# zju3dv/pats

Hardware: AMD Instinct MI355X
Metric: image-pairs/sec (coarse+fine OT) on 640x480 MegaDepth; OT iters/sec per pair (higher is better)
Workload: dtype f32 (contractions: fp32 operands split into fp16 hi + lo, three exact-product MFMA passes, fp32 accumulate)

## Files before the change

include/pats_amd.h:

```cpp
#ifndef PATS_AMD_H
#define PATS_AMD_H

#include <stddef.h>
#include <stdint.h>

#ifdef __cplusplus
extern "C" {
#endif

typedef void* pats_stream_t;

enum {
    PATS_OK = 0,
    PATS_ERR_INVALID = 1,
    PATS_ERR_UNSUPPORTED = 2,
    PATS_ERR_LAUNCH = 3,
    PATS_ERR_NO_DEVICE = 4
};

enum { PATS_SINKHORN_AUTO = 0, PATS_SINKHORN_LOG = 1, PATS_SINKHORN_KERNEL = 2 };

const char* pats_version(void);
#define PATS_ABI_VERSION 8
int pats_abi_version(void);
const char* pats_last_error(void);
int pats_device_count(void);
int pats_set_sinkhorn_mode(int mode);
int pats_set_fine_fused(int on);

int pats_set_third_gather(int mode);

int pats_sinkhorn_fallbacks(int64_t* count, int reset);

int pats_cost_f32(const float* d0, const float* d1, int64_t batch, int D, int n, int m, float* out,
                  pats_stream_t stream);

size_t pats_sinkhorn_workspace_bytes(int64_t batch, int M, int N);
int pats_sinkhorn_f32(const float* Z, int64_t batch, int M, int N, const float* log_mu,
                      const float* log_nu, int iters, float* out, void* workspace,
                      size_t workspace_bytes, pats_stream_t stream);

size_t pats_ot_workspace_bytes(int64_t batch, int M, int N);
int pats_log_optimal_transport_f32(const float* scores, int64_t batch, int m, int n,
                                   const float* alpha, const float* ns, int iters, float* Z,
                                   void* workspace, size_t workspace_bytes, pats_stream_t stream);

size_t pats_ot2_workspace_bytes(int64_t batch, int m, int n);
int pats_log_optimal_transport2_flags_f32(const float* scores, int64_t batch, int m, int n,
                                          const float* one, const float* ns, int iters, float bias_k,
                                          float* Z, uint8_t* col_nomatch, void* workspace,
                                          size_t workspace_bytes, pats_stream_t stream);
int pats_log_optimal_transport2_f32(const float* scores, int64_t batch, int m, int n,
                                    const float* one, const float* ns, int iters, float bias_k,
                                    float* Z, void* workspace, size_t workspace_bytes,
                                    pats_stream_t stream);

int pats_cost_ot_f32(const float* d0, const float* d1, int64_t batch, int D, int n, int m,
                     int variant, const float* scalar, const float* ns, int iters, float bias_k,
                     float* Z, void* workspace, size_t workspace_bytes, pats_stream_t stream);
size_t pats_cost_ot_workspace_bytes(int64_t batch, int D, int n, int m, int variant);
int pats_cost_ot_flags_f32(const float* d0, const float* d1, int64_t batch, int D, int n, int m,
                           int variant, const float* scalar, const float* ns, int iters, float bias_k,
                           float* Z, uint8_t* col_nomatch, void* workspace, size_t workspace_bytes,
                           pats_stream_t stream);

int pats_set_cost_ot_mid_event(void* event);

int pats_cost_ot_flags_counted_f32(const float* d0, const float* d1, int64_t batch_cap, const int64_t* batch_dev,
                                   int D, int n, int m, int variant, const float* scalar, const float* ns, int iters,
                                   float bias_k, float* Z, uint8_t* col_nomatch, void* workspace,
                                   size_t workspace_bytes, pats_stream_t stream);

int pats_colmass_sqrt_f32(const float* Z, int64_t batch, int M, int N, float* out,
                          pats_stream_t stream);
int pats_colmass_flags_f32(const float* Z, int64_t batch, int M, int N, float* out, uint8_t* col_nomatch,
                           pats_stream_t stream);
int pats_dustbin_bias_inplace_f32(float* Z, int64_t batch, int M, int N, float k,
                                  pats_stream_t stream);
int pats_exp_f32(const float* Z, int64_t count, float* out, pats_stream_t stream);

int pats_argmax_f32(const float* Z, int64_t batch, int M, int N, int64_t* row_arg,
                    int64_t* col_arg, pats_stream_t stream);

int pats_iterative_expand_f32(const float* P, int input_is_log, int64_t batch, int M, int N,
                              const float* scalex, const float* scaley, int lim3, int h, int w,
                              float lower_bound, int iter_num, float* whole_cost, float* core_cost,
                              float* average_point, float* x_scale, float* y_scale, int64_t* bound,
                              uint8_t* row_nomatch, pats_stream_t stream);

int pats_iterative_expand_counted_f32(const float* P, int input_is_log, int64_t batch_cap, const int64_t* batch_dev,
                                      int M, int N, const float* scalex, const float* scaley, int lim3, int h, int w,
                                      float lower_bound, int iter_num, float* whole_cost, float* core_cost,
                                      float* average_point, float* x_scale, float* y_scale, int64_t* bound,
                                      uint8_t* row_nomatch, pats_stream_t stream);

int pats_split_patches(const int32_t* sum_cycle_host, int height, int width, int max_once_used,
                       int64_t* second_layer_set, int64_t* third_layer_set);
int pats_split_patches_device(const int32_t* sum_cycle, int64_t pairs, int height, int width,
                              int max_once_used, int64_t* second_layer_set, int64_t* third_layer_set,
                              int32_t* cycle_num, pats_stream_t stream);

int pats_compute_imgs_bounds_f32(const float* x_scale, const float* y_scale,
                                 const float* average_point, const uint8_t* if_nomatching, int Np,
                                 int height, int width, int img, int64_t* bound5, int64_t* K_out,
                                 float* x_scale_new, float* y_scale_new, float* average_new,
                                 pats_stream_t stream);

int pats_left_crops_f32(const float* left, int n_img, int H, int W, const int64_t* bound5, int64_t K,
                        int height, int width, float* out, pats_stream_t stream);

int pats_compute_imgs_bounds_batch_f32(const float* x_scale, const float* y_scale, const float* average_point,
                                       const uint8_t* if_nomatching, int n_img, int Np, int height, int width,
                                       int64_t* bound5, int64_t* K_img, int64_t* K_total, float* x_scale_new,
                                       float* y_scale_new, float* average_new, pats_stream_t stream);
int pats_left_crops_counted_f32(const float* left, int n_img, int H, int W, const int64_t* bound5,
                                int64_t K_cap, const int64_t* K_dev, int height, int width, float* out,
                                pats_stream_t stream);

int pats_tensor_resize_f32(const float* input, int n_img, int C, int Hp, int Wp,
                           const int64_t* bound, int64_t K, float* out, int32_t* status,
                           pats_stream_t stream);
int pats_tensor_resize_hwc_f32(const float* right, int n_img, int H, int W, int margin,
                               const int64_t* bound, int64_t K, float* out, int32_t* status,
                               pats_stream_t stream);
int pats_tensor_resize_hwc_counted_f32(const float* right, int n_img, int H, int W, int margin,
                                       const int64_t* bound, int64_t K_cap, const int64_t* K_dev, float* out,
                                       int32_t* status, pats_stream_t stream);

int pats_compute_result_f32(const float* scores, int input_is_log, int64_t P, const float* scale_x,
                            const float* scale_y, const int64_t* p_s, const int64_t* p_t,
                            int outdoor, float* mkpts0_f, float* mkpts1_f, float* whole_loss,
                            float* label, uint8_t* if_matching1, pats_stream_t stream);
int pats_compute_result_ws_f32(const float* scores, int input_is_log, int64_t P, const float* scale_x,
                               const float* scale_y, const int64_t* p_s, const int64_t* p_t,
                               int outdoor, float* mkpts0_f, float* mkpts1_f, float* whole_loss,
                               float* label, uint8_t* if_matching1, void* workspace, size_t workspace_bytes,
                               pats_stream_t stream);

int pats_fine_descriptors_f32(const float* feat0, const float* feat1, const float* feat2,
                              const float* title, const float* rubbish, int64_t B, float* desc,
                              pats_stream_t stream);

int pats_fine_descriptors_counted_f32(const float* feat0, const float* feat1, const float* feat2,
                                      const float* title, const float* rubbish, int64_t B_cap,
                                      const int64_t* B_dev, int channels_last, float* desc, pats_stream_t stream);

int pats_third_descriptors_f32(const float* feat_f0, const float* feat_f1, const float* mkpts0_c,
                               const float* mkpts1_c, const int64_t* b_ids, const float* kenc,
                               const float* rubbish, int64_t P, int64_t B, float* out0, float* out1,
                               int64_t* p_s_out, int64_t* p_t_out, pats_stream_t stream);

int pats_third_level_f32(const float* feat0, const float* feat1, int64_t P, int D, const float* scale,
                         const float* scale_x, const float* scale_y, const int64_t* p_s,
                         const int64_t* p_t, int iters, int outdoor, float* mkpts0_f, float* mkpts1_f,
                         float* label, uint8_t* if_matching1, float* Z_out, pats_stream_t stream);

int pats_third_descriptors_counted_f32(const float* feat_f0, const float* feat_f1, const float* mkpts0_c,
                                       const float* mkpts1_c, const int64_t* b_ids, const float* kenc,
                                       const float* rubbish, int64_t P_cap, const int64_t* P_dev, int64_t B,
                                       float* out0, float* out1, int64_t* p_s_out, int64_t* p_t_out,
                                       pats_stream_t stream);
int pats_third_level_counted_f32(const float* feat0, const float* feat1, int64_t P_cap, const int64_t* P_dev, int D,
                                 const float* scale, const float* scale_x, const float* scale_y, const int64_t* p_s,
                                 const int64_t* p_t, int iters, int outdoor, float* mkpts0_f, float* mkpts1_f,
                                 float* label, uint8_t* if_matching1, pats_stream_t stream);

int pats_fine_descriptors_nhwc_f32(const float* feat0, const float* feat1, const float* feat2,
                                   const float* title, const float* rubbish, int64_t B, float* desc,
                                   pats_stream_t stream);
int pats_third_descriptors_nhwc_f32(const float* feat_f0, const float* feat_f1, const float* mkpts0_c,
                                    const float* mkpts1_c, const int64_t* b_ids, const float* kenc,
                                    const float* rubbish, int64_t P_cap, const int64_t* P_dev, int64_t B,
                                    float* out0, float* out1, int64_t* p_s_out, int64_t* p_t_out,
                                    pats_stream_t stream);

typedef enum { PATS_MAP_F32 = 0, PATS_MAP_F16 = 1, PATS_MAP_BF16 = 2 } pats_map_dtype_t;
int pats_fine_descriptors_typed(const void* feat0, const void* feat1, const void* feat2, pats_map_dtype_t dtype,
                                int channels_last, const float* title, const float* rubbish, int64_t B_cap,
                                const int64_t* B_dev, float* desc, pats_stream_t stream);
int pats_third_descriptors_typed(const void* feat_f0, const void* feat_f1, pats_map_dtype_t dtype, int channels_last,
                                 const float* mkpts0_c, const float* mkpts1_c, const int64_t* b_ids, const float* kenc,
                                 const float* rubbish, int64_t P_cap, const int64_t* P_dev, int64_t B, float* out0,
                                 float* out1, int64_t* p_s_out, int64_t* p_t_out, pats_stream_t stream);
// ... 206 lines not shown
```

pats_amd/_lib.py:

```python
import ctypes
import os

_HERE = os.path.dirname(os.path.abspath(__file__))
LIB_PATH = os.path.join(_HERE, "libpats_amd.so")
if os.environ.get("PATS_AMD_DIAG_LIB", "") not in ("", "0"):
    _sfx = os.environ["PATS_AMD_DIAG_LIB"]
    LIB_PATH = os.path.join(_HERE, "libpats_amd_diag%s.so" % ("" if _sfx == "1" else _sfx))

c_void_p, c_int, c_i64, c_f, c_size = (ctypes.c_void_p, ctypes.c_int, ctypes.c_int64, ctypes.c_float,
                                       ctypes.c_size_t)

ABI_VERSION = 8



class PairTable(ctypes.Structure):
    _fields_ = [("pairs", ctypes.c_int64), ("shape_host", c_void_p), ("cell_base_host", c_void_p), ("shape", c_void_p),
                ("cell_base", c_void_p), ("img_base", c_void_p)]


_TAB = ctypes.POINTER(PairTable)


class CropFormat(ctypes.Structure):
    _fields_ = [("dtype", ctypes.c_int32), ("layout", ctypes.c_int32), ("normalize", ctypes.c_int32),
                ("mean", ctypes.c_float * 3), ("std", ctypes.c_float * 3)]


_FMT = ctypes.POINTER(CropFormat)

SIGNATURES = {
    "pats_version": (ctypes.c_char_p, []),
    "pats_abi_version": (c_int, []),
    "pats_last_error": (ctypes.c_char_p, []),
    "pats_device_count": (c_int, []),
    "pats_set_sinkhorn_mode": (c_int, [c_int]),
    "pats_set_fine_fused": (c_int, [c_int]),
    "pats_set_third_gather": (c_int, [c_int]),
    "pats_sinkhorn_fallbacks": (c_int, [ctypes.POINTER(ctypes.c_int64), c_int]),
    "pats_set_gnn_redo_mode": (c_int, [c_int]),
    "pats_gnn_overflows": (c_int, [ctypes.POINTER(ctypes.c_int64), c_int]),
    "pats_cost_f32": (c_int, [c_void_p, c_void_p, c_i64, c_int, c_int, c_int, c_void_p, c_void_p]),
    "pats_sinkhorn_workspace_bytes": (c_size, [c_i64, c_int, c_int]),
    "pats_sinkhorn_f32": (c_int, [c_void_p, c_i64, c_int, c_int, c_void_p, c_void_p, c_int, c_void_p,
                                  c_void_p, c_size, c_void_p]),
    "pats_ot_workspace_bytes": (c_size, [c_i64, c_int, c_int]),
    "pats_log_optimal_transport_f32": (c_int, [c_void_p, c_i64, c_int, c_int, c_void_p, c_void_p, c_int,
                                               c_void_p, c_void_p, c_size, c_void_p]),
    "pats_ot2_workspace_bytes": (c_size, [c_i64, c_int, c_int]),
    "pats_log_optimal_transport2_f32": (c_int, [c_void_p, c_i64, c_int, c_int, c_void_p, c_void_p, c_int,
                                                c_f, c_void_p, c_void_p, c_size, c_void_p]),
    "pats_cost_ot_f32": (c_int, [c_void_p, c_void_p, c_i64, c_int, c_int, c_int, c_int, c_void_p,
                                 c_void_p, c_int, c_f, c_void_p, c_void_p, c_size, c_void_p]),
    "pats_cost_ot_flags_f32": (c_int, [c_void_p, c_void_p, c_i64, c_int, c_int, c_int, c_int, c_void_p,
                                       c_void_p, c_int, c_f, c_void_p, c_void_p, c_void_p, c_size, c_void_p]),
    "pats_set_cost_ot_mid_event": (c_int, [c_void_p]),
    "pats_cost_ot_flags_counted_f32": (c_int, [c_void_p, c_void_p, c_i64, c_void_p, c_int, c_int, c_int, c_int, c_void_p,
                                               c_void_p, c_int, c_f, c_void_p, c_void_p, c_void_p, c_size, c_void_p]),
    "pats_iterative_expand_counted_f32": (c_int, [c_void_p, c_int, c_i64, c_void_p, c_int, c_int, c_void_p, c_void_p, c_int,
                                                  c_int, c_int, c_f, c_int, c_void_p, c_void_p, c_void_p,
                                                  c_void_p, c_void_p, c_void_p, c_void_p, c_void_p]),
    "pats_fine_descriptors_counted_f32": (c_int, [c_void_p, c_void_p, c_void_p, c_void_p, c_void_p, c_i64, c_void_p, c_int,
                                                  c_void_p, c_void_p]),
    "pats_log_optimal_transport2_flags_f32": (c_int, [c_void_p, c_i64, c_int, c_int, c_void_p, c_void_p, c_int,
                                                      c_f, c_void_p, c_void_p, c_void_p, c_size, c_void_p]),
    "pats_colmass_flags_f32": (c_int, [c_void_p, c_i64, c_int, c_int, c_void_p, c_void_p, c_void_p]),
    "pats_cost_ot_workspace_bytes": (c_size, [c_i64, c_int, c_int, c_int, c_int]),
    "pats_colmass_sqrt_f32": (c_int, [c_void_p, c_i64, c_int, c_int, c_void_p, c_void_p]),
    "pats_dustbin_bias_inplace_f32": (c_int, [c_void_p, c_i64, c_int, c_int, c_f, c_void_p]),
    "pats_exp_f32": (c_int, [c_void_p, c_i64, c_void_p, c_void_p]),
    "pats_argmax_f32": (c_int, [c_void_p, c_i64, c_int, c_int, c_void_p, c_void_p, c_void_p]),
    "pats_iterative_expand_f32": (c_int, [c_void_p, c_int, c_i64, c_int, c_int, c_void_p, c_void_p, c_int,
                                          c_int, c_int, c_f, c_int, c_void_p, c_void_p, c_void_p,
                                          c_void_p, c_void_p, c_void_p, c_void_p, c_void_p]),
    "pats_split_patches": (c_int, [c_void_p, c_int, c_int, c_int, c_void_p, c_void_p]),
    "pats_split_patches_device": (c_int, [c_void_p, c_i64, c_int, c_int, c_int, c_void_p, c_void_p, c_void_p, c_void_p]),
    "pats_compute_imgs_bounds_batch_f32": (c_int, [c_void_p, c_void_p, c_void_p, c_void_p, c_int, c_int, c_int, c_int,
                                                   c_void_p, c_void_p, c_void_p, c_void_p, c_void_p, c_void_p, c_void_p]),
    "pats_left_crops_counted_f32": (c_int, [c_void_p, c_int, c_int, c_int, c_void_p, c_i64, c_void_p, c_int, c_int,
                                            c_void_p, c_void_p]),
    "pats_tensor_resize_hwc_counted_f32": (c_int, [c_void_p, c_int, c_int, c_int, c_int, c_void_p, c_i64, c_void_p,
                                                   c_void_p, c_void_p, c_void_p]),
    "pats_compute_imgs_bounds_f32": (c_int, [c_void_p, c_void_p, c_void_p, c_void_p, c_int, c_int, c_int,
                                             c_int, c_void_p, c_void_p, c_void_p, c_void_p, c_void_p,
                                             c_void_p]),
    "pats_left_crops_f32": (c_int, [c_void_p, c_int, c_int, c_int, c_void_p, c_i64, c_int, c_int, c_void_p,
                                    c_void_p]),
    "pats_tensor_resize_f32": (c_int, [c_void_p, c_int, c_int, c_int, c_int, c_void_p, c_i64, c_void_p,
                                       c_void_p, c_void_p]),
    "pats_tensor_resize_hwc_f32": (c_int, [c_void_p, c_int, c_int, c_int, c_int, c_void_p, c_i64,
                                           c_void_p, c_void_p, c_void_p]),
    "pats_compute_result_f32": (c_int, [c_void_p, c_int, c_i64, c_void_p, c_void_p, c_void_p, c_void_p,
                                        c_int, c_void_p, c_void_p, c_void_p, c_void_p, c_void_p,
                                        c_void_p]),
    "pats_compute_result_ws_f32": (c_int, [c_void_p, c_int, c_i64, c_void_p, c_void_p, c_void_p, c_void_p,
                                           c_int, c_void_p, c_void_p, c_void_p, c_void_p, c_void_p,
                                           c_void_p, c_size, c_void_p]),
    "pats_fine_descriptors_f32": (c_int, [c_void_p, c_void_p, c_void_p, c_void_p, c_void_p, c_i64, c_void_p, c_void_p]),
    "pats_third_descriptors_f32": (c_int, [c_void_p, c_void_p, c_void_p, c_void_p, c_void_p, c_void_p, c_void_p,
                                           c_i64, c_i64, c_void_p, c_void_p, c_void_p, c_void_p, c_void_p]),
    "pats_third_level_f32": (c_int, [c_void_p, c_void_p, c_i64, c_int, c_void_p, c_void_p, c_void_p, c_void_p,
                                     c_void_p, c_int, c_int, c_void_p, c_void_p, c_void_p, c_void_p, c_void_p,
                                     c_void_p]),
    "pats_third_descriptors_counted_f32": (c_int, [c_void_p, c_void_p, c_void_p, c_void_p, c_void_p, c_void_p, c_void_p,
                                                   c_i64, c_void_p, c_i64, c_void_p, c_void_p, c_void_p, c_void_p, c_void_p]),
    "pats_fine_descriptors_nhwc_f32": (c_int, [c_void_p, c_void_p, c_void_p, c_void_p, c_void_p, c_i64, c_void_p, c_void_p]),
    "pats_third_descriptors_nhwc_f32": (c_int, [c_void_p, c_void_p, c_void_p, c_void_p, c_void_p, c_void_p, c_void_p,
                                                c_i64, c_void_p, c_i64, c_void_p, c_void_p, c_void_p, c_void_p, c_void_p]),
    "pats_fine_descriptors_typed": (c_int, [c_void_p, c_void_p, c_void_p, c_int, c_int, c_void_p, c_void_p, c_i64, c_void_p,
                                            c_void_p, c_void_p]),
    "pats_third_descriptors_typed": (c_int, [c_void_p, c_void_p, c_int, c_int, c_void_p, c_void_p, c_void_p, c_void_p, c_void_p,
                                             c_i64, c_void_p, c_i64, c_void_p, c_void_p, c_void_p, c_void_p, c_void_p]),
    "pats_third_level_counted_f32": (c_int, [c_void_p, c_void_p, c_i64, c_void_p, c_int, c_void_p, c_void_p, c_void_p,
                                             c_void_p, c_void_p, c_int, c_int, c_void_p, c_void_p, c_void_p, c_void_p,
                                             c_void_p]),
    "pats_cost_typed": (c_int, [c_void_p, c_void_p, c_int, c_i64, c_int, c_int, c_int, c_void_p, c_void_p]),
    "pats_cost_ot_typed": (c_int, [c_void_p, c_void_p, c_int, c_i64, c_void_p, c_int, c_int, c_int, c_int, c_void_p, c_void_p,
                                   c_int, c_f, c_void_p, c_void_p, c_void_p, c_size, c_void_p]),
    "pats_third_level_typed": (c_int, [c_void_p, c_void_p, c_int, c_i64, c_void_p, c_int, c_void_p, c_void_p, c_void_p, c_void_p,
                                       c_void_p, c_int, c_int, c_void_p, c_void_p, c_void_p, c_void_p, c_void_p, c_void_p]),
    "pats_chunk_rows_workspace_bytes": (c_size, [c_i64, c_int]),
    "pats_chunk_rows_device": (c_int, [c_void_p, c_i64, c_int, c_int, c_int, c_int, c_i64] + [c_void_p] * 13 +
                               [c_size, c_void_p]),
    "pats_profile_marker": (c_int, [c_int, c_void_p]),
    "pats_stream_create_cu_mask": (c_int, [c_void_p, c_int, c_void_p]),
    "pats_stream_destroy": (c_int, [c_void_p]),
    "pats_merge_batch_workspace_bytes": (c_size, [c_i64, c_int, c_int]),
    "pats_merge_patches_batch": (c_int, [c_int, c_int, c_i64, c_int, c_int, c_i64] + [c_void_p] * 7 + [c_int, c_void_p, c_void_p,
                                         c_size, c_void_p]),
    "pats_merge_patches_chunks": (c_int, [c_int, c_int, c_int, c_int, c_i64, c_int, c_int, c_i64, c_i64] + [c_void_p] * 7 +
                                  [c_int, c_void_p, c_void_p, c_size, c_void_p]),
    "pats_chunk_fine_tail_workspace_bytes": (c_size, [c_i64, c_i64, c_int, c_int]),
    "pats_chunk_fine_tail_f32": (c_int, [c_void_p, c_void_p, c_i64, c_void_p, c_void_p, c_int, c_f, c_void_p, c_void_p, c_int, c_int, c_int,
                                         c_i64, c_int, c_int, c_i64] + [c_void_p] * 5 + [c_int] + [c_void_p] * 16 + [c_void_p, c_size, c_void_p]),
    "pats_chunk_third_tail_workspace_bytes": (c_size, [c_i64, c_int, c_int]),
    "pats_chunk_third_tail_f32": (c_int, [c_void_p, c_void_p, c_i64, c_void_p, c_void_p, c_void_p, c_void_p, c_int, c_int, c_void_p, c_void_p,
                                          c_i64, c_void_p, c_int, c_int, c_void_p, c_void_p, c_void_p] + [c_void_p] * 10 +
                                  [c_void_p, c_size, c_void_p]),
    "pats_get_result_chunks_f32": (c_int, [c_int, c_i64, c_void_p, c_void_p, c_i64, c_void_p, c_void_p, c_void_p,
                                           ctypes.POINTER(c_int), ctypes.POINTER(c_int), c_void_p, c_void_p, c_void_p,
                                           c_void_p, c_void_p, c_i64, c_void_p, c_void_p, c_size, c_void_p]),
    "pats_merge_workspace_bytes": (c_size, [c_i64, c_int, c_int, c_int]),
    "pats_merge_patches": (c_int, [c_int, c_i64, c_void_p, c_int, c_int, c_int, c_void_p, c_void_p, c_void_p,
                                   c_void_p, c_void_p, c_size, c_void_p]),
    "pats_compact_workspace_bytes": (c_size, [c_i64]),
    "pats_third_inputs_f32": (c_int, [c_void_p, c_void_p, c_i64, c_void_p, c_void_p, c_void_p, c_i64, c_void_p,
                                      c_void_p, c_size, c_void_p]),
    "pats_refine_scatter_f32": (c_int, [c_void_p, c_void_p, c_void_p, c_void_p, c_int, c_i64, c_i64, c_void_p,
                                        c_void_p, c_void_p, c_size, c_void_p]),
    "pats_attention_f32": (c_int, [c_void_p, c_void_p, c_void_p, c_i64, c_int, c_int, c_int, c_int, c_void_p, c_void_p,
                                   c_void_p]),
    "pats_attentional_propagation_workspace_bytes": (c_size, [c_i64, c_int, c_int, c_int]),
    "pats_attentional_propagation_f32": (c_int, [c_void_p, c_void_p, c_i64, c_int, c_int, c_int, c_int, c_void_p, c_int, c_f,
                                                 c_void_p, c_void_p, c_void_p, c_size, c_void_p]),
    "pats_propagation_packed_bytes": (c_size, [c_int, c_int]),
    "pats_propagation_pack_f32": (c_int, [c_void_p, c_int, c_int, c_void_p, c_size, c_void_p]),
    "pats_attentional_propagation_packed_f32": (c_int, [c_void_p, c_void_p, c_i64, c_int, c_int, c_int, c_int, c_void_p, c_void_p,
                                                        c_int, c_f, c_void_p, c_void_p, c_void_p, c_size, c_void_p]),
    "pats_attentional_gnn_packed_workspace_bytes": (c_size, [c_i64, c_int, c_int, c_int]),
    "pats_attentional_gnn_packed_f32": (c_int, [c_void_p, c_void_p, c_i64, c_void_p, c_i64, c_int, c_int, c_int, c_int, c_void_p, c_void_p,
                                                c_void_p, c_f, c_void_p, c_void_p, c_void_p, c_size, c_void_p]),
    "pats_attentional_propagation_packed_counted_f32": (c_int, [c_void_p, c_void_p, c_i64, c_void_p, c_i64, c_int, c_int, c_int, c_int,
                                                                c_void_p, c_void_p, c_int, c_f, c_void_p, c_void_p, c_void_p, c_size,
                                                                c_void_p]),
    "pats_matches_by_pair_workspace_bytes": (c_size, [c_int, c_i64]),
    "pats_matches_by_pair_f32": (c_int, [c_void_p, c_void_p, c_void_p, c_void_p, c_void_p, c_void_p, c_int, c_i64, c_int,
                                         c_void_p, c_void_p, c_void_p, c_void_p, c_size, c_void_p]),
    "pats_matches_by_pair_summary_f32": (c_int, [c_void_p, c_void_p, c_void_p, c_void_p, c_void_p, c_void_p, c_int, c_i64, c_int,
                                                 c_void_p, c_void_p, c_void_p, c_void_p, c_void_p, c_void_p, c_size, c_void_p]),
    "pats_chunk_rows_ragged": (c_int, [_TAB, c_void_p, c_int, c_int, c_i64] + [c_void_p] * 14 + [c_size, c_void_p]),
    "pats_compute_imgs_bounds_ragged_f32": (c_int, [_TAB] + [c_void_p] * 10 + [c_void_p]),
    "pats_left_crops_ragged_f32": (c_int, [_TAB, c_void_p, c_void_p, c_i64, c_void_p, c_void_p, c_void_p]),
    "pats_tensor_resize_hwc_ragged_f32": (c_int, [_TAB, c_void_p, c_int, c_void_p, c_i64, c_void_p, c_void_p, c_void_p, c_void_p]),
    "pats_left_crops_typed": (c_int, [_TAB, c_void_p, c_int, c_int, c_int, c_int, c_int, c_int, c_void_p, c_i64, c_void_p,
                                      _FMT, c_void_p, c_void_p]),
    "pats_tensor_resize_hwc_typed": (c_int, [_TAB, c_void_p, c_int, c_int, c_int, c_int, c_int, c_void_p, c_i64, c_void_p, _FMT,
                                             c_void_p, c_void_p, c_void_p]),
    "pats_tensor_resize_typed": (c_int, [c_void_p, c_int, c_int, c_int, c_int, c_int, c_void_p, c_i64, c_void_p, _FMT, c_void_p,
                                         c_void_p, c_void_p]),
    "pats_merge_ragged_workspace_bytes": (c_size, [c_i64]),
    "pats_merge_patches_ragged": (c_int, [_TAB, c_int, c_int, c_i64] + [c_void_p] * 8 + [c_int, c_void_p, c_void_p, c_size, c_void_p]),
    "pats_get_result_chunks_ragged_f32": (c_int, [_TAB, c_int, c_void_p, c_void_p, c_i64, c_void_p, c_void_p, c_void_p,
                                                  ctypes.POINTER(c_int), c_void_p, c_void_p, c_void_p, c_void_p, c_void_p, c_i64,
                                                  c_void_p, c_void_p, c_size, c_void_p]),
    "pats_matches_by_row_pair_summary_f32": (c_int, [c_void_p, c_void_p, c_void_p, c_void_p, c_void_p, c_void_p, c_int, c_i64,
                                                     c_void_p, c_void_p, c_void_p, c_void_p, c_void_p, c_void_p, c_size, c_void_p]),
    "pats_conv1x1_workspace_bytes": (c_size, []),
    "pats_conv1x1_f32": (c_int, [c_void_p, c_void_p, c_void_p, c_i64, c_int, c_int, c_int, c_void_p, c_void_p, c_void_p,
                                 c_void_p, c_void_p, c_size, c_void_p]),
    "pats_bn_fold_workspace_bytes": (c_size, [c_int]),
    "pats_bn_fold_f32": (c_int, [c_void_p, c_i64, c_int, c_int, c_void_p, c_void_p, c_f, c_void_p, c_void_p, c_void_p,
# ... 41 lines not shown
```

pats_amd/csrc/expand.hip:

```cpp
#include "common.hpp"
#include "third_device.hpp"

namespace pats {

struct ExpandArgs {
    const float* P;
    int input_is_log;
    int64_t rows_total;
    int M, N;
    const float* scalex;
    const float* scaley;
    int lim3, h, w;
    float lower_bound;
    int iter_num;
    float *whole_cost, *core_cost, *average_point, *x_scale, *y_scale;
    int64_t* bound;
    uint8_t* row_nomatch;
    const int64_t* live;
};

__device__ __forceinline__ float range_val(int d, int k) { return k <= d ? (float)k : 1e7f; }

__device__ __forceinline__ int clamp_seq(float f, int wh, int S) {
    return (f >= 0.f && f <= (float)(wh - 1)) ? (int)f : S;
// ... 80 lines not shown
    int up = max0 / a.lim3, down = up, left = max0 % a.lim3, right = left;
    int bd0 = 0, bd1 = 0, sb0 = 0, sb1 = 0;
    float last_sum = ES(max0);

    for (int it = 0; it < a.iter_num; ++it) {
        sb0 = bd0; sb1 = bd1;
        const float off[4] = {(float)(left + up * width - width),
                              (float)(left + down * width + width),
                              (float)(left + up * width - 1),
                              (float)(right + up * width + 1)};
        float es[4], nm[4], sc[4];
        float vcell[4];
        int scell[4];
#pragma unroll
        for (int d = 0; d < 4; ++d) {
            float e = 0.f, q = 0.f, c = 0.f;
            auto cell = [&](int k) {
                const float f = d < 2 ? range_val(sb1, k) + off[d] : range_val(sb0, k) * (float)width + off[d];
                const int s = clamp_seq(f, wh, S);
                const float v = ES(s);
                e += v;
                if (SMALL) { vcell[d] = v; scell[d] = s; }
                else {
                    q += (v > a.lower_bound) ? EOPP(s) : ZERO_F;
                    c += ESC(s);
                }
            };
            if (SMALL) { vcell[d] = 0.f; scell[d] = S; if (t < width) cell(t); }
            else for (int k = t; k < width; k += 16) cell(k);
            es[d] = row16_sum(e);
            if (!SMALL) { nm[d] = row16_sum(q); sc[d] = row16_sum(c); }
        }
        if (up == 0) es[0] = ZERO_F;
        if (down == height - 1) es[1] = ZERO_F;
        if (left == 0) es[2] = ZERO_F;
        if (right == width - 1) es[3] = ZERO_F;
        int arg = 0;
        float mx = es[0];
#pragma unroll
        for (int d = 1; d < 4; ++d)
            if (es[d] > mx) { mx = es[d]; arg = d; }
        float mnm;
        if (SMALL) {
            float v = vcell[0];
            int sidx = scell[0];
#pragma unroll
            for (int d = 1; d < 4; ++d)
                if (arg == d) { v = vcell[d]; sidx = scell[d]; }
            const float q = (t < width) ? ((v > a.lower_bound) ? EOPP(sidx) : ZERO_F) : 0.f;
            mnm = row16_sum(q);
        } else {
            mnm = nm[0];
#pragma unroll
            for (int d = 1; d < 4; ++d)
                if (arg == d) mnm = nm[d];
        }
        (void)sc;
        float add_sum = ZERO_F, add_nm = ZERO_F;
        if (mx > a.lower_bound) {
            up -= (arg == 0);
            down += (arg == 1);
            left -= (arg == 2);
            right += (arg == 3);
            add_sum = mx;
            add_nm = mnm;
        }
        bd0 = down - up;
        bd1 = right - left;
        last_sum = last_sum + add_sum;
        last_nomatching = last_nomatching + add_nm;
    }
    const bool if_core_exist = (bd0 > 1) && (bd1 > 1);

    float e4, s4;
    {
        const float eoff[4] = {(float)(left + up * width), (float)(left + down * width),
                               (float)(left + up * width), (float)(right + up * width)};
        float ed[4], sd[4];
#pragma unroll
        for (int d = 0; d < 4; ++d) {
            float e = 0.f, c = 0.f;
            auto cell = [&](int k) {
                const float f = d < 2 ? range_val(sb1, k) + eoff[d]
                                      : range_val(sb0, k) * (float)width + eoff[d];
                const int s = clamp_seq(f, wh, S);
                e += ES(s);
                c += ESC(s);
            };
            if (SMALL) { if (t < width) cell(t); }
            else for (int k = t; k < width; k += 16) cell(k);
            ed[d] = row16_sum(e);
            sd[d] = row16_sum(c);
        }
        e4 = (ed[0] + ed[1]) + (ed[2] + ed[3]);
        s4 = (sd[0] + sd[1]) + (sd[2] + sd[3]);
    }

    float wx = 0.f, wy = 0.f, sumx = 0.f, sumy = 0.f, ws = 0.f, so = 0.f;
    const int q16 = 16 / a.w, r16 = 16 - q16 * a.w;
    int pyi = t / a.w, pxi = t - pyi * a.w;
    const bool no_cell = up > (n - 1) / a.w || left > a.w - 1;
    for (int p = t; p < n; p += 16, pyi += q16, pxi += r16) {
        if (pxi >= a.w) { pxi -= a.w; ++pyi; }
        const bool crit = pyi >= up && pyi <= down && pxi >= left && pxi <= right;
        if (!__any(crit || no_cell)) continue;
        const float fx = sx[p], fy = sy[p];
        float ox = ZERO_F, oy = ZERO_F;
        if (crit) {
            const float root = sqrtf(prow[p] + 1e-7f);
            ox = root / fx;
            oy = root / fy;
        }
        wx += ox * (float)pxi;
        wy += oy * (float)pyi;
        sumx += ox;
        sumy += oy;
        const float o = ox * oy;
        ws += o * (fx * fy);
        so += o;
    }
    wx = row16_sum(wx); wy = row16_sum(wy); sumx = row16_sum(sumx); sumy = row16_sum(sumy);
    ws = row16_sum(ws); so = row16_sum(so);

    if (t == 0 && active) {
        const int corner[4] = {up * width + left, up * width + right, down * width + left,
                               down * width + right};
        float cps = 0.f, css = 0.f;
#pragma unroll
        for (int q = 0; q < 4; ++q) {
            int s = corner[q];
            if (!(s >= 0)) s = S;
            if (!(s <= wh - 1)) s = S;
            cps += ES(s);
            css += ESC(s);
        }
        const float core_scale_sum = the_scale - s4 + css;
        const float core_sum = last_sum - e4 + cps;
        a.core_cost[gr] = (if_core_exist && !if_nomatching)
                              ? fabsf((core_sum - core_scale_sum) / the_scale) : ZERO_F;
        a.whole_cost[gr] = if_nomatching ? ZERO_F
            : (fabsf(the_scale - last_sum) + last_nomatching / 4.0f) / the_scale;
        a.average_point[gr * 2 + 1] = wx / sumx + 0.5f;
        a.average_point[gr * 2 + 0] = wy / sumy + 0.5f;
        const float average_scale = sqrtf(ws / so);
        a.x_scale[gr] = 1.0f / (average_scale / 1.0f);
        a.y_scale[gr] = 1.0f / (average_scale * 1.0f);
        a.bound[gr * 4 + 0] = up;
        a.bound[gr * 4 + 1] = down;
        a.bound[gr * 4 + 2] = left;
        a.bound[gr * 4 + 3] = right;
    }
}

}

using namespace pats;

static int expand_impl(const float* P, int input_is_log, int64_t batch, int M, int N, const float* scalex, const float* scaley,
                       int lim3, int h, int w, float lower_bound, int iter_num, float* whole_cost, float* core_cost,
                       float* average_point, float* x_scale, float* y_scale, int64_t* bound, uint8_t* row_nomatch,
                       const int64_t* live, pats_stream_t stream);

extern "C" int pats_iterative_expand_f32(const float* P, int input_is_log, int64_t batch, int M,
                                         int N, const float* scalex, const float* scaley, int lim3,
                                         int h, int w, float lower_bound, int iter_num,
                                         float* whole_cost, float* core_cost, float* average_point,
                                         float* x_scale, float* y_scale, int64_t* bound,
                                         uint8_t* row_nomatch, pats_stream_t stream) {
    return expand_impl(P, input_is_log, batch, M, N, scalex, scaley, lim3, h, w, lower_bound, iter_num, whole_cost, core_cost,
                       average_point, x_scale, y_scale, bound, row_nomatch, nullptr, stream);
}

extern "C" int pats_iterative_expand_counted_f32(const float* P, int input_is_log, int64_t batch_cap, const int64_t* batch_dev,
                                                 int M, int N, const float* scalex, const float* scaley, int lim3, int h, int w,
                                                 float lower_bound, int iter_num, float* whole_cost, float* core_cost,
                                                 float* average_point, float* x_scale, float* y_scale, int64_t* bound,
                                                 uint8_t* row_nomatch, pats_stream_t stream) {
    PATS_REQUIRE(batch_dev, "iterative_expand_counted: null count");
    return expand_impl(P, input_is_log, batch_cap, M, N, scalex, scaley, lim3, h, w, lower_bound, iter_num, whole_cost, core_cost,
                       average_point, x_scale, y_scale, bound, row_nomatch, batch_dev, stream);
}

static int expand_impl(const float* P, int input_is_log, int64_t batch, int M, int N, const float* scalex, const float* scaley,
                       int lim3, int h, int w, float lower_bound, int iter_num, float* whole_cost, float* core_cost,
                       float* average_point, float* x_scale, float* y_scale, int64_t* bound, uint8_t* row_nomatch,
                       const int64_t* live, pats_stream_t stream) {
    PATS_REQUIRE(batch >= 0 && M > 1 && N > 1 && h > 0 && w > 0 && lim3 > 0 && iter_num >= 1,
                 "iterative_expand: bad argument");
    PATS_REQUIRE(h * w == N - 1, "iterative_expand: grid %dx%d does not match %d target columns", h,
                 w, N - 1);
    if (batch == 0) return PATS_OK;
    PATS_REQUIRE(P && scalex && scaley && whole_cost && core_cost && average_point && x_scale &&
                     y_scale && bound, "iterative_expand: null pointer");
    ExpandArgs a{P, input_is_log, batch * (int64_t)(M - 1), M, N, scalex, scaley, lim3, h, w,
                 lower_bound, iter_num, whole_cost, core_cost, average_point, x_scale, y_scale, bound, row_nomatch, live};
    int rows_per_wg = 16;
    size_t lds = 2 * (size_t)rows_per_wg * (size_t)(N + 3) * sizeof(float);
    if (lds > 48 * 1024) {
        rows_per_wg = 4;
        lds = 2 * (size_t)rows_per_wg * (size_t)(N + 3) * sizeof(float);
    }
    PATS_REQUIRE(lds <= 64 * 1024, "iterative_expand: N=%d too large", N);
    const int64_t blocks = ceil_div(a.rows_total, rows_per_wg);
    if (h <= 16 && w <= 16)
        hipLaunchKernelGGL(expand_kernel<true>, dim3((unsigned)blocks), dim3(16 * rows_per_wg), lds, as_stream(stream), a);
    else
        hipLaunchKernelGGL(expand_kernel<false>, dim3((unsigned)blocks), dim3(16 * rows_per_wg), lds, as_stream(stream), a);
    return check_launch("expand_kernel");
}
```

pats_amd/ops.py:

```python
import ctypes

import numpy as np
import torch

from . import _lib

_L = _lib.lib
_check = _lib.check
_L()


_raw_stream = getattr(torch._C, "_cuda_getCurrentRawStream", None)


def _stream():
    if _raw_stream is not None:
        return ctypes.c_void_p(_raw_stream(torch.cuda.current_device()))
    return ctypes.c_void_p(torch.cuda.current_stream().cuda_stream)


def _dev(t, name, dtype=torch.float32):
    if not isinstance(t, torch.Tensor):
        raise TypeError("%s must be a torch.Tensor" % name)
    if not t.is_cuda:
        raise RuntimeError("pats_amd: %s is on %s; the HIP path needs a GPU tensor (no CPU fallback)"
                           % (name, t.device))
    if t.dtype != dtype:
        raise RuntimeError("pats_amd: %s must be %s, got %s" % (name, dtype, t.dtype))
    return t.contiguous()


def _map(t, name, dtype=torch.float32):
    if not isinstance(t, torch.Tensor):
        raise TypeError("%s must be a torch.Tensor" % name)
    if not t.is_cuda:
        raise RuntimeError("pats_amd: %s is on %s; the HIP path needs a GPU tensor (no CPU fallback)" % (name, t.device))
    if t.dtype != dtype:
        raise RuntimeError("pats_amd: %s must be %s, got %s" % (name, dtype, t.dtype))
    if t.dim() == 4 and not t.is_contiguous() and t.is_contiguous(memory_format=torch.channels_last):
        return t, True
    return t.contiguous(), False


_MAP_DTYPES = {torch.float32: 0, torch.float16: 1, torch.bfloat16: 2}


def _maps_any(tensors, names):
    for t, name in zip(tensors, names):
        if not isinstance(t, torch.Tensor):
            raise TypeError("%s must be a torch.Tensor" % name)
        if t.dtype not in _MAP_DTYPES:
            raise RuntimeError("pats_amd: %s must be float32, float16 or bfloat16, got %s" % (name, t.dtype))
    dtypes = {t.dtype for t in tensors}
    if dtypes == {torch.float32}:
        return [_map(t, n) for t, n in zip(tensors, names)], _MAP_DTYPES[torch.float32]
    if len(dtypes) != 1:
        return [_map(t.float(), n) for t, n in zip(tensors, names)], _MAP_DTYPES[torch.float32]
    dt = tensors[0].dtype
    maps = [_map(t, n, dt) for t, n in zip(tensors, names)]
    if len({cl for _, cl in maps}) != 1:
        maps = [(t.contiguous(), False) for t, _ in maps]
    align = 16 if maps[0][1] else 4
    if any(t.data_ptr() % align for t, _ in maps):
        return [_map(t.float(), n) for t, n in zip(tensors, names)], _MAP_DTYPES[torch.float32]
    return maps, _MAP_DTYPES[dt]


def _descs_any(tensors, names):
    for t, name in zip(tensors, names):
        if not isinstance(t, torch.Tensor):
            raise TypeError("%s must be a torch.Tensor" % name)
        if t.dtype not in _MAP_DTYPES:
            raise RuntimeError("pats_amd: %s must be float32, float16 or bfloat16, got %s" % (name, t.dtype))
    dtypes = {t.dtype for t in tensors}
    if len(dtypes) == 1 and torch.float32 not in dtypes:
        dt = tensors[0].dtype
        descs = [_dev(t, n, dt) for t, n in zip(tensors, names)]
        if not any(t.data_ptr() % t.element_size() for t in descs):
            return descs, _MAP_DTYPES[dt]
    return [_dev(t.float(), n) for t, n in zip(tensors, names)], _MAP_DTYPES[torch.float32]


def _ptr(t):
    return ctypes.c_void_p(t.data_ptr()) if t is not None else ctypes.c_void_p(0)


_WS = {}
_WS_MAX = 64 << 20
_WS_ON = [False]


class workspace_cache:

    def __enter__(self):
        self.prev = _WS_ON[0]
        _WS_ON[0] = True

    def __exit__(self, *exc):
        _WS_ON[0] = self.prev


def _workspace(nbytes, device):
    n = max(int(nbytes), 1)
    if not _WS_ON[0] or n > _WS_MAX or _raw_stream is None or torch.cuda.is_current_stream_capturing():
        return torch.empty(n, dtype=torch.uint8, device=device)
    key = (device.index, _raw_stream(torch.cuda.current_device()))
    t = _WS.get(key)
    if t is None or t.numel() < n:
        t = _WS[key] = torch.empty(min(_WS_MAX, max(2 * n, 1 << 20)), dtype=torch.uint8, device=device)
    return t


def _scalar_dev(x, device):
    if isinstance(x, torch.Tensor):
        return x.detach().reshape(1).to(device=device, dtype=torch.float32)
    return torch.full((1,), float(x), dtype=torch.float32, device=device)


def set_sinkhorn_mode(mode):
    names = {"auto": 0, "log": 1, "kernel": 2}
    prev = _L().pats_set_sinkhorn_mode(names[mode])
    return {v: k for k, v in names.items()}[prev]


def set_fine_fused(on):
    return bool(_L().pats_set_fine_fused(1 if on else 0))


def set_third_gather(mode):
    modes = {"tile": 0, "point": 1}
    if mode not in modes:
        raise ValueError("set_third_gather: mode must be 'tile' or 'point'")
    prev = _L().pats_set_third_gather(modes[mode])
    return {v: k for k, v in modes.items()}.get(prev, "tile")


def sinkhorn_fallbacks(reset=True):
    import ctypes
    n = ctypes.c_int64(0)
    rc = _L().pats_sinkhorn_fallbacks(ctypes.byref(n), 1 if reset else 0)
    if rc != 0:
        raise RuntimeError(_L().pats_last_error().decode())
    return int(n.value)


def set_gnn_redo(mode):
    names = {"inline": 0, "deferred": 1}
    prev = _L().pats_set_gnn_redo_mode(names[mode])
    return {v: k for k, v in names.items()}[prev]


def gnn_overflows(reset=True):
    n = ctypes.c_int64(0)
    _check(_L().pats_gnn_overflows(ctypes.byref(n), 1 if reset else 0), "gnn_overflows")
    return bool(n.value)


def cost(mdesc0, mdesc1, out=None):
    (d0, d1), code = _descs_any([mdesc0, mdesc1], ["mdesc0", "mdesc1"])
    b, D, n = d0.shape
    if d1.shape[0] != b or d1.shape[1] != D:
        raise RuntimeError("cost: descriptor shapes %s / %s do not match" % (tuple(d0.shape), tuple(d1.shape)))
    m = d1.shape[2]
    if out is None:
        out = torch.empty((b, n, m), dtype=torch.float32, device=d0.device)
    elif tuple(out.shape) != (b, n, m) or out.dtype != torch.float32 or not out.is_contiguous() or out.device != d0.device:
        raise RuntimeError("cost: out must be a contiguous float32 [%d, %d, %d] tensor on %s" % (b, n, m, d0.device))
    if code:
        _check(_L().pats_cost_typed(_ptr(d0), _ptr(d1), code, b, D, n, m, _ptr(out), _stream()), "cost")
    else:
        _check(_L().pats_cost_f32(_ptr(d0), _ptr(d1), b, D, n, m, _ptr(out), _stream()), "cost")
    return out


def log_sinkhorn_iterations(Z, log_mu, log_nu, iters: int):
    Z, log_mu, log_nu = _dev(Z, "Z"), _dev(log_mu, "log_mu"), _dev(log_nu, "log_nu")
    b, M, N = Z.shape
    if tuple(log_mu.shape) != (b, M) or tuple(log_nu.shape) != (b, N):
        raise RuntimeError("log_sinkhorn_iterations: marginal shapes do not match Z")
    out = torch.empty_like(Z)
    nb = _L().pats_sinkhorn_workspace_bytes(b, M, N)
    ws = _workspace(nb, Z.device)
    _check(_L().pats_sinkhorn_f32(_ptr(Z), b, M, N, _ptr(log_mu), _ptr(log_nu), int(iters), _ptr(out),
                                  _ptr(ws), nb, _stream()), "log_sinkhorn_iterations")
    return out


def log_optimal_transport(scores, alpha, ns, iters: int):
    scores = _dev(scores, "scores")
    b, m, n = scores.shape
    ns = _dev(ns, "ns")
    if ns.numel() != b * n:
        raise RuntimeError("log_optimal_transport: ns must have %d entries per batch" % n)
    ns = ns.reshape(b, n)
    a = _scalar_dev(alpha, scores.device)
    Z = torch.empty((b, m + 1, n + 1), dtype=torch.float32, device=scores.device)
    nb = _L().pats_ot_workspace_bytes(b, m + 1, n + 1)
    ws = _workspace(nb, scores.device)
    _check(_L().pats_log_optimal_transport_f32(_ptr(scores), b, m, n, _ptr(a), _ptr(ns), int(iters),
                                               _ptr(Z), _ptr(ws), nb, _stream()), "log_optimal_transport")
    return Z


def log_optimal_transport2(scores, one, ns, iters: int, bias_k: float = 0.0):
    scores = _dev(scores, "scores")
    b, m, n = scores.shape
    ns = _dev(ns, "ns")
    if ns.numel() != b * (n - 1):
        raise RuntimeError("log_optimal_transport2: ns must have %d entries per batch" % (n - 1))
    ns = ns.reshape(b, n - 1)
    o = _scalar_dev(one, scores.device)
    Z = torch.empty((b, m, n), dtype=torch.float32, device=scores.device)
    nb = _L().pats_ot2_workspace_bytes(b, m, n)
    ws = _workspace(nb, scores.device)
    _check(_L().pats_log_optimal_transport2_f32(_ptr(scores), b, m, n, _ptr(o), _ptr(ns), int(iters),
                                                float(bias_k), _ptr(Z), _ptr(ws), nb, _stream()),
           "log_optimal_transport2")
    return Z


def set_cost_ot_mid_event(event):
    h = None if event is None else ctypes.c_void_p(event.cuda_event)
    _check(_L().pats_set_cost_ot_mid_event(h), "set_cost_ot_mid_event")


def cost_ot(mdesc0, mdesc1, variant, scalar, ns, iters: int, bias_k: float = 0.0, return_flags=False, count=None):
    (d0, d1), code = _descs_any([mdesc0, mdesc1], ["mdesc0", "mdesc1"])
    b, D, n = d0.shape
    m = d1.shape[2]
    ns = _dev(_widen(ns), "ns").reshape(b, m if variant == 1 else m - 1)
    s = _scalar_dev(scalar, d0.device)
    shape = (b, n + 1, m + 1) if variant == 1 else (b, n, m)
    Z = torch.empty(shape, dtype=torch.float32, device=d0.device)
    nb = _L().pats_cost_ot_workspace_bytes(b, D, n, m, variant)
    ws = _workspace(nb, d0.device)
    if return_flags:
        if variant != 2:
            raise RuntimeError("cost_ot: return_flags needs variant 2 (the coarse level gets them from colmass_sqrt)")
        flags = torch.empty((b, m - 1), dtype=torch.bool, device=d0.device)
        cnt = _dev(count, "count", torch.int64) if count is not None else None
        if code:
            _check(_L().pats_cost_ot_typed(_ptr(d0), _ptr(d1), code, b, _ptr(cnt) if cnt is not None else None, D, n, m,
                                           int(variant), _ptr(s), _ptr(ns), int(iters), float(bias_k), _ptr(Z),
                                           _ptr(flags.view(torch.uint8)), _ptr(ws), nb, _stream()), "cost_ot")
            return Z, flags
        if count is not None:
            _check(_L().pats_cost_ot_flags_counted_f32(_ptr(d0), _ptr(d1), b, _ptr(cnt), D, n, m, int(variant), _ptr(s), _ptr(ns),
                                                       int(iters), float(bias_k), _ptr(Z), _ptr(flags.view(torch.uint8)), _ptr(ws),
                                                       nb, _stream()), "cost_ot")
            return Z, flags
        _check(_L().pats_cost_ot_flags_f32(_ptr(d0), _ptr(d1), b, D, n, m, int(variant), _ptr(s), _ptr(ns), int(iters),
                                           float(bias_k), _ptr(Z), _ptr(flags.view(torch.uint8)), _ptr(ws), nb, _stream()),
               "cost_ot")
        return Z, flags
    if count is not None:
        raise RuntimeError("cost_ot: count needs return_flags=True (the fine level's counted launch)")
    if code:
        _check(_L().pats_cost_ot_typed(_ptr(d0), _ptr(d1), code, b, None, D, n, m, int(variant), _ptr(s), _ptr(ns), int(iters),
                                       float(bias_k), _ptr(Z), None, _ptr(ws), nb, _stream()), "cost_ot")
        return Z
    _check(_L().pats_cost_ot_f32(_ptr(d0), _ptr(d1), b, D, n, m, int(variant), _ptr(s), _ptr(ns),
                                 int(iters), float(bias_k), _ptr(Z), _ptr(ws), nb, _stream()), "cost_ot")
    return Z


def colmass_sqrt(Z, return_flags=False):
    Z = _dev(Z, "Z")
    b, M, N = Z.shape
    out = torch.empty((b, N - 1), dtype=torch.float32, device=Z.device)
    if return_flags:
        flags = torch.empty((b, N - 1), dtype=torch.bool, device=Z.device)
        _check(_L().pats_colmass_flags_f32(_ptr(Z), b, M, N, _ptr(out), _ptr(flags.view(torch.uint8)), _stream()),
               "colmass_sqrt")
        return out, flags
    _check(_L().pats_colmass_sqrt_f32(_ptr(Z), b, M, N, _ptr(out), _stream()), "colmass_sqrt")
    return out


def dustbin_bias_(Z, k):
    if not Z.is_contiguous():
        raise RuntimeError("dustbin_bias_: Z must be contiguous (in-place op)")
    _dev(Z, "Z")
    b, M, N = Z.shape
    _check(_L().pats_dustbin_bias_inplace_f32(_ptr(Z), b, M, N, float(k), _stream()), "dustbin_bias_")
    return Z


# ... 1348 lines not shown
```

Measured before the change: 1924.

## Add packed 4-lane-per-row expand kernel with shared opposite-row staging

```diff
diff --git a/include/pats_amd.h b/include/pats_amd.h
--- a/include/pats_amd.h
+++ b/include/pats_amd.h
@@ -29,6 +29,8 @@
 int pats_set_fine_fused(int on);
 
 int pats_set_third_gather(int mode);
+
+int pats_set_expand_variant(int variant);
 
 int pats_sinkhorn_fallbacks(int64_t* count, int reset);
 
diff --git a/pats_amd/_lib.py b/pats_amd/_lib.py
--- a/pats_amd/_lib.py
+++ b/pats_amd/_lib.py
@@ -37,6 +37,7 @@
     "pats_set_sinkhorn_mode": (c_int, [c_int]),
     "pats_set_fine_fused": (c_int, [c_int]),
     "pats_set_third_gather": (c_int, [c_int]),
+    "pats_set_expand_variant": (c_int, [c_int]),
     "pats_sinkhorn_fallbacks": (c_int, [ctypes.POINTER(ctypes.c_int64), c_int]),
     "pats_set_gnn_redo_mode": (c_int, [c_int]),
     "pats_gnn_overflows": (c_int, [ctypes.POINTER(ctypes.c_int64), c_int]),
diff --git a/pats_amd/csrc/expand.hip b/pats_amd/csrc/expand.hip
--- a/pats_amd/csrc/expand.hip
+++ b/pats_amd/csrc/expand.hip
@@ -256,9 +256,262 @@
     }
 }
 
+__device__ __forceinline__ float quad_sum(const float (&s)[4]) {
+    float q = (s[0] + s[1]) + (s[2] + s[3]);
+    q += dpp_f<DPP_QUAD_XOR1>(q);
+    q += dpp_f<DPP_QUAD_XOR2>(q);
+    return q;
+}
+__device__ __forceinline__ void quad_argmax(float& v, int& i) {
+    argmax_step<DPP_QUAD_XOR1>(v, i);
+    argmax_step<DPP_QUAD_XOR2>(v, i);
+}
+
+__global__ void __launch_bounds__(256)
+expand_packed_kernel(ExpandArgs a, int ld) {
+    extern __shared__ __attribute__((aligned(16))) float sm[];
+    const int j = threadIdx.x & 3, slot = threadIdx.x >> 2;
+    const int t0 = 4 * j;
+    const int ROWS_PER_WG = blockDim.x >> 2;
+    const int M = a.M, N = a.N, m = M - 1, n = N - 1;
+    int64_t rows_total = a.rows_total;
+    if (a.live) {
+        const int64_t lv = *a.live * m;
+        rows_total = lv < rows_total ? lv : rows_total;
+        if ((int64_t)blockIdx.x * ROWS_PER_WG >= rows_total) return;
+    }
+    const int64_t gr_raw = (int64_t)blockIdx.x * ROWS_PER_WG + slot;
+    const bool active = gr_raw < rows_total;
+    const int64_t gr = active ? gr_raw : rows_total - 1;
+    const int64_t b = gr / m;
+    const int r = (int)(gr - b * m);
+    float* prow = sm + (size_t)slot * ld;
+    float* popp = sm + (size_t)ROWS_PER_WG * ld + (size_t)slot * ld;
+    const float* Pb = a.P + b * (int64_t)M * N;
+    const float* src = Pb + (int64_t)r * N;
+    const float* oppsrc = Pb + (int64_t)(M - 1) * N;
+    const float* sx = a.scalex + b * (int64_t)n;
+    const float* sy = a.scaley + b * (int64_t)n;
+    const int64_t g0 = (int64_t)blockIdx.x * ROWS_PER_WG;
+    const int64_t glast = min(g0 + ROWS_PER_WG - 1, rows_total - 1);
+    const int64_t b0 = g0 / m;
+    const bool shared_opp = glast / m - b0 <= 1;
+    if (shared_opp) {
+        popp = sm + (size_t)ROWS_PER_WG * ld + (size_t)(b - b0) * ld;
+        for (int e = threadIdx.x; e < 2 * N; e += blockDim.x) {
+            const int which = e >= N, c = e - which * N;
+            const int64_t bb = min(b0 + which, (int64_t)(rows_total - 1) / m);
+            const float o = a.P[bb * (int64_t)M * N + (int64_t)(M - 1) * N + c];
+            sm[(size_t)ROWS_PER_WG * ld + (size_t)which * ld + c] = a.input_is_log ? expf(o) : o;
+        }
+    }
+    float fv = -INFINITY, bv = -INFINITY;
+    int fi = 0x7fffffff, bi = 0x7fffffff;
+    float rs[4] = {0.f, 0.f, 0.f, 0.f};
+    for (int c0 = t0; c0 < N; c0 += 16) {
+#pragma unroll
+        for (int i = 0; i < 4; ++i) {
+            const int c = c0 + i;
+            if (c < N) {
+                const float x0 = src[c];
+                if (x0 > fv || fi == 0x7fffffff) { fv = x0; fi = c; }
+                const float x = a.input_is_log ? expf(x0) : x0;
+                prow[c] = x;
+                rs[i] += x;
+                if (c < N - 1 && (x > bv || bi == 0x7fffffff)) { bv = x; bi = c; }
+                if (!shared_opp) {
+                    const float o = oppsrc[c];
+                    popp[c] = a.input_is_log ? expf(o) : o;
+                }
+            }
+        }
+    }
+    if (a.row_nomatch) {
+        quad_argmax(fv, fi);
+        if (j == 0 && active) a.row_nomatch[gr] = fi == N - 1;
+    }
+    if (j == 0) { prow[N] = ZERO_F; popp[N] = ZERO_F; prow[N + 1] = 0.f; popp[N + 1] = 0.f; }
+    wg_barrier();
+
+    const int width = a.h > a.w ? a.h : a.w;
+    const int height = (a.h * a.w) / width;
+    const int wh = width * height, S = wh + 1;
+    auto ESC = [&](int idx) { return idx < n ? sx[idx] * sy[idx] : ZERO_F; };
+    int fill[4], kw[4];
+#pragma unroll
+    for (int i = 0; i < 4; ++i) { fill[i] = t0 + i < width ? S : S + 1; kw[i] = (t0 + i) * width; }
+
+    quad_argmax(bv, bi);
+    const float the_scale = quad_sum(rs);
+    const int max0 = bi;
+    const bool if_nomatching = (prow[n] > bv ? n : bi) == m;
+    float last_nomatching = popp[max0];
+    int up = max0 / a.lim3, down = up, left = max0 % a.lim3, right = left;
+    int bd0 = 0, bd1 = 0, sb0 = 0, sb1 = 0;
+    float last_sum = prow[max0];
+
+    auto strip_index = [&](int d, int base, int i) {
+        const int k = t0 + i;
+        const int s = d < 2 ? base + k : base + kw[i];
+        const bool real = k <= min(d < 2 ? sb1 : sb0, width - 1) && (unsigned)s < (unsigned)wh;
+        return real ? s : fill[i];
+    };
+
+    for (int it = 0; it < a.iter_num; ++it) {
+        sb0 = bd0; sb1 = bd1;
+        const int base[4] = {left + up * width - width, left + down * width + width, left + up * width - 1,
+                             right + up * width + 1};
+        float es[4];
+        int hit[4][4];
+#pragma unroll
+        for (int d = 0; d < 4; ++d) {
+            float e[4];
+#pragma unroll
+            for (int i = 0; i < 4; ++i) {
+                const int s = strip_index(d, base[d], i);
+                e[i] = prow[s];
+                hit[d][i] = e[i] > a.lower_bound ? s : fill[i];
+            }
+            es[d] = quad_sum(e);
+        }
+        if (up == 0) es[0] = ZERO_F;
+        if (down == height - 1) es[1] = ZERO_F;
+        if (left == 0) es[2] = ZERO_F;
+        if (right == width - 1) es[3] = ZERO_F;
+        int arg = 0;
+        float mx = es[0];
+#pragma unroll
+        for (int d = 1; d < 4; ++d)
+            if (es[d] > mx) { mx = es[d]; arg = d; }
+        float q[4];
+#pragma unroll
+        for (int i = 0; i < 4; ++i) {
+            int s = hit[0][i];
+#pragma unroll
+            for (int d = 1; d < 4; ++d)
+                if (arg == d) s = hit[d][i];
+            q[i] = popp[s];
+        }
+        const float mnm = quad_sum(q);
+        float add_sum = ZERO_F, add_nm = ZERO_F;
+        if (mx > a.lower_bound) {
+            up -= (arg == 0);
+            down += (arg == 1);
+            left -= (arg == 2);
+            right += (arg == 3);
+            add_sum = mx;
+            add_nm = mnm;
+        }
+        bd0 = down - up;
+        bd1 = right - left;
+        last_sum = last_sum + add_sum;
+        last_nomatching = last_nomatching + add_nm;
+    }
+    const bool if_core_exist = (bd0 > 1) && (bd1 > 1);
+
+    float e4, s4;
+    {
+        const int ebase[4] = {left + up * width, left + down * width, left + up * width, right + up * width};
+        float ed[4], sd[4];
+#pragma unroll
+        for (int d = 0; d < 4; ++d) {
+            float e[4], c[4];
+#pragma unroll
+            for (int i = 0; i < 4; ++i) {
+                const int s = strip_index(d, ebase[d], i);
+                e[i] = prow[s];
+                c[i] = s < wh ? sx[s] * sy[s] : (s == S ? ZERO_F : 0.f);
+            }
+            ed[d] = quad_sum(e);
+            sd[d] = quad_sum(c);
+        }
+        e4 = (ed[0] + ed[1]) + (ed[2] + ed[3]);
+        s4 = (sd[0] + sd[1]) + (sd[2] + sd[3]);
+    }
+
+    float wx[4] = {0.f, 0.f, 0.f, 0.f}, wy[4] = {0.f, 0.f, 0.f, 0.f}, sumx[4] = {0.f, 0.f, 0.f, 0.f},
+          sumy[4] = {0.f, 0.f, 0.f, 0.f}, ws[4] = {0.f, 0.f, 0.f, 0.f}, so[4] = {0.f, 0.f, 0.f, 0.f};
+    const int q16 = 16 / a.w, r16 = 16 - q16 * a.w;
+    int pyi[4], pxi[4];
+#pragma unroll
+    for (int i = 0; i < 4; ++i) { pyi[i] = (t0 + i) / a.w; pxi[i] = (t0 + i) - pyi[i] * a.w; }
+    const bool no_cell = up > (n - 1) / a.w || left > a.w - 1;
+    const int rowshift = threadIdx.x & 48;
+    for (int p0 = t0; p0 - t0 < n; p0 += 16) {
+        bool crit[4], any = false;
+#pragma unroll
+        for (int i = 0; i < 4; ++i) {
+            if (pxi[i] >= a.w) { pxi[i] -= a.w; ++pyi[i]; }
+            crit[i] = pyi[i] >= up && pyi[i] <= down && pxi[i] >= left && pxi[i] <= right;
+            any = any || (p0 + i < n && (crit[i] || no_cell));
+        }
+        const bool band = ((__builtin_amdgcn_ballot_w64(any) >> rowshift) & 0xffffull) != 0ull;
+#pragma unroll
+        for (int i = 0; i < 4; ++i) {
+            const int p = p0 + i;
+            if (band && p < n) {
+                const float fx = sx[p], fy = sy[p];
+                float ox = ZERO_F, oy = ZERO_F;
+                if (crit[i]) {
+                    const float root = sqrtf(prow[p] + 1e-7f);
+                    ox = root / fx;
+                    oy = root / fy;
+                }
+                wx[i] += ox * (float)pxi[i];
+                wy[i] += oy * (float)pyi[i];
+                sumx[i] += ox;
+                sumy[i] += oy;
+                const float o = ox * oy;
+                ws[i] += o * (fx * fy);
+                so[i] += o;
+            }
+            pyi[i] += q16;
+            pxi[i] += r16;
+        }
+    }
+    const float wxs = quad_sum(wx), wys = quad_sum(wy), sumxs = quad_sum(sumx), sumys = quad_sum(sumy);
+    const float wss = quad_sum(ws), sos = quad_sum(so);
+
+    if (j == 0 && active) {
+        const int corner[4] = {up * width + left, up * width + right, down * width + left,
+                               down * width + right};
+        float cps = 0.f, css = 0.f;
+#pragma unroll
+        for (int q = 0; q < 4; ++q) {
+            int s = corner[q];
+            if (!(s >= 0)) s = S;
+            if (!(s <= wh - 1)) s = S;
+            cps += prow[s];
+            css += ESC(s);
+        }
+        const float core_scale_sum = the_scale - s4 + css;
+        const float core_sum = last_sum - e4 + cps;
+        a.core_cost[gr] = (if_core_exist && !if_nomatching)
+                              ? fabsf((core_sum - core_scale_sum) / the_scale) : ZERO_F;
+        a.whole_cost[gr] = if_nomatching ? ZERO_F
+            : (fabsf(the_scale - last_sum) + last_nomatching / 4.0f) / the_scale;
+        a.average_point[gr * 2 + 1] = wxs / sumxs + 0.5f;
+        a.average_point[gr * 2 + 0] = wys / sumys + 0.5f;
+        const float average_scale = sqrtf(wss / sos);
+        a.x_scale[gr] = 1.0f / (average_scale / 1.0f);
+        a.y_scale[gr] = 1.0f / (average_scale * 1.0f);
+        a.bound[gr * 4 + 0] = up;
+        a.bound[gr * 4 + 1] = down;
+        a.bound[gr * 4 + 2] = left;
+        a.bound[gr * 4 + 3] = right;
+    }
+}
+
 }
 
 using namespace pats;
+
+static int g_expand_variant = 0;
+extern "C" int pats_set_expand_variant(int variant) {
+    const int prev = g_expand_variant;
+    if (variant == 0 || variant == 1) g_expand_variant = variant;
+    return prev;
+}
 
 static int expand_impl(const float* P, int input_is_log, int64_t batch, int M, int N, const float* scalex, const float* scaley,
                        int lim3, int h, int w, float lower_bound, int iter_num, float* whole_cost, float* core_cost,
@@ -298,6 +551,16 @@
                      y_scale && bound, "iterative_expand: null pointer");
     ExpandArgs a{P, input_is_log, batch * (int64_t)(M - 1), M, N, scalex, scaley, lim3, h, w,
                  lower_bound, iter_num, whole_cost, core_cost, average_point, x_scale, y_scale, bound, row_nomatch, live};
+    if (h <= 16 && w <= 16 && g_expand_variant == 0) {
+        const int ld = (N + 3) | 1;
+        int rows = 64;
+        auto bytes = [&](int rws) { return (size_t)(rws + (M - 1 >= rws - 1 ? 2 : rws)) * (size_t)ld * sizeof(float); };
+        while (rows > 4 && bytes(rows) > 64 * 1024) rows /= 2;
+        PATS_REQUIRE(bytes(rows) <= 64 * 1024, "iterative_expand: N=%d too large", N);
+        const int64_t blocks = ceil_div(a.rows_total, rows);
+        hipLaunchKernelGGL(expand_packed_kernel, dim3((unsigned)blocks), dim3(4 * rows), bytes(rows), as_stream(stream), a, ld);
+        return check_launch("expand_packed_kernel");
+    }
     int rows_per_wg = 16;
     size_t lds = 2 * (size_t)rows_per_wg * (size_t)(N + 3) * sizeof(float);
     if (lds > 48 * 1024) {
diff --git a/pats_amd/ops.py b/pats_amd/ops.py
--- a/pats_amd/ops.py
+++ b/pats_amd/ops.py
@@ -133,6 +133,14 @@
         raise ValueError("set_third_gather: mode must be 'tile' or 'point'")
     prev = _L().pats_set_third_gather(modes[mode])
     return {v: k for k, v in modes.items()}.get(prev, "tile")
+
+
+def set_expand_variant(variant):
+    variants = {"packed": 0, "row16": 1}
+    if variant not in variants:
+        raise ValueError("set_expand_variant: variant must be 'packed' or 'row16'")
+    prev = _L().pats_set_expand_variant(variants[variant])
+    return {v: k for k, v in variants.items()}.get(prev, "packed")
 
 
 def sinkhorn_fallbacks(reset=True):
```

Result: no change. 1956 (median of 2 runs) (+1.6%).
